# microsoft/DiskANN

Hardware: NVIDIA H100
Metric: QPS @ recall@10>=0.95, 1Mx128 f32 L2 (Vamana R=64 greedy search, batch 10K) (higher is better)
Workload: dtype f32

## Files before the change

### diskann_b200/csrc/search_common.cuh

```cuda
#pragma once

#include "distance_device.cuh"

namespace dab {

constexpr uint32_t kEmptyV2 = 0xFFFFFFFFu;
constexpr uint32_t kFlagV2 = 0x80000000u;

__device__ __forceinline__ uint32_t bucket_of(uint32_t id, uint32_t n_buckets) { return __umulhi(id * 0x9E3779B1u, n_buckets); }


__device__ __forceinline__ uint32_t first_unvisited(const uint32_t* qi, uint32_t from, uint32_t lim, int lane) {
    for (uint32_t b = from & ~31u; b < lim; b += 32) {
        const uint32_t i = b + lane;
        const bool u = i >= from && i < lim && !(qi[i] & kFlagV2);
        const unsigned m = __ballot_sync(kFull, u);
        if (m) return b + __ffs(m) - 1;
    }
    return lim;
}

template <int QT>
__device__ __forceinline__ void merge_round(float* qd, uint32_t* qi, uint32_t cap, uint32_t& size, uint32_t& cursor_lo,
                                            const uint32_t* cid, const float* cd, uint32_t c0, uint32_t m, int lane) {
    const uint32_t j = (uint32_t)lane;
    const float dj = j < m ? cd[c0 + j] : __int_as_float(0x7FC00000);
    const uint32_t idj = j < m ? cid[c0 + j] : 0;
    const float worst = size == cap ? qd[cap - 1] : __int_as_float(0x7F800000);
    const bool valid = j < m && dj == dj && !(worst < dj);
    const unsigned vm = __ballot_sync(kFull, valid);
    if (!vm) return;
    uint32_t lo = 0, hi = size;
    while (__any_sync(kFull, lo < hi)) {
        const uint32_t mid = (lo + hi) >> 1;
        if (lo < hi) {
            if (qd[mid] < dj) lo = mid + 1;
            else hi = mid;
        }
    }
    float od[QT];
    uint32_t oi[QT], sh[QT];
#pragma unroll
    for (int t = 0; t < QT; ++t) {
        const uint32_t e = (uint32_t)t * 32 + lane;
        od[t] = e < size ? qd[e] : __int_as_float(0x7F800000);
        oi[t] = e < size ? qi[e] : kEmptyV2;
        sh[t] = 0;
    }
    uint32_t rn = 0;
    unsigned it = vm;
    while (it) {
        const int i = __ffs(it) - 1;
        it &= it - 1;
        const float di = __shfl_sync(kFull, dj, i);
        rn += (di < dj || (di == dj && (uint32_t)i > j)) ? 1u : 0u;
#pragma unroll
        for (int t = 0; t < QT; ++t) sh[t] += di <= od[t] ? 1u : 0u;
    }
    const uint32_t pos = lo + rn;
    const bool keep_new = valid && pos < cap;
    __syncwarp();
#pragma unroll
    for (int t = 0; t < QT; ++t) {
        const uint32_t e = (uint32_t)t * 32 + lane;
        const uint32_t ne = e + sh[t];
        if (e < size && sh[t] != 0 && ne < cap) {
            qd[ne] = od[t];
            qi[ne] = oi[t];
        }
    }
    if (keep_new) {
        qd[pos] = dj;
        qi[pos] = idj;
    }
    size = min(cap, size + (uint32_t)__popc(vm));
    cursor_lo = min(cursor_lo, __reduce_min_sync(kFull, keep_new ? pos : 0xFFFFFFFFu));
    __syncwarp();
}

template <int QT>
__device__ __forceinline__ void merge_round_chunked(float* qd, uint32_t* qi, uint32_t cap, uint32_t& size, uint32_t& cursor_lo,
                                                    const uint32_t* cid, const float* cd, uint32_t c0, uint32_t m, int lane) {
    const uint32_t j = (uint32_t)lane;
    const float dj = j < m ? cd[c0 + j] : __int_as_float(0x7FC00000);
    const uint32_t idj = j < m ? cid[c0 + j] : 0;
    const float worst = size == cap ? qd[cap - 1] : __int_as_float(0x7F800000);
    const bool valid = j < m && dj == dj && !(worst < dj);
    const unsigned vm = __ballot_sync(kFull, valid);
    if (!vm) return;
    uint32_t lo = 0, hi = size;
    while (__any_sync(kFull, lo < hi)) {
        const uint32_t mid = (lo + hi) >> 1;
        if (lo < hi) {
            if (qd[mid] < dj) lo = mid + 1;
            else hi = mid;
        }
    }
    uint32_t rn = 0;
    for (unsigned it = vm; it;) {
        const int i = __ffs(it) - 1;
        it &= it - 1;
        const float di = __shfl_sync(kFull, dj, i);
        rn += (di < dj || (di == dj && (uint32_t)i > j)) ? 1u : 0u;
    }
    const uint32_t pos = lo + rn;
    const bool keep_new = valid && pos < cap;
    __syncwarp();
#pragma unroll 1
    for (uint32_t c = (size + QT * 32 - 1) / (QT * 32); c-- > 0;) {
        const uint32_t e0 = c * QT * 32;
        float od[QT];
        uint32_t oi[QT], sh[QT];
#pragma unroll
        for (int t = 0; t < QT; ++t) {
            const uint32_t e = e0 + (uint32_t)t * 32 + lane;
            od[t] = e < size ? qd[e] : __int_as_float(0x7F800000);
            oi[t] = e < size ? qi[e] : kEmptyV2;
            sh[t] = 0;
        }
        for (unsigned it = vm; it;) {
            const int i = __ffs(it) - 1;
            it &= it - 1;
            const float di = __shfl_sync(kFull, dj, i);
#pragma unroll
            for (int t = 0; t < QT; ++t) sh[t] += di <= od[t] ? 1u : 0u;
        }
        __syncwarp();
#pragma unroll
        for (int t = 0; t < QT; ++t) {
            const uint32_t e = e0 + (uint32_t)t * 32 + lane;
            const uint32_t ne = e + sh[t];
            if (e < size && sh[t] != 0 && ne < cap) {
                qd[ne] = od[t];
                qi[ne] = oi[t];
            }
        }
        __syncwarp();
    }
    if (keep_new) {
        qd[pos] = dj;
        qi[pos] = idj;
    }
    size = min(cap, size + (uint32_t)__popc(vm));
    cursor_lo = min(cursor_lo, __reduce_min_sync(kFull, keep_new ? pos : 0xFFFFFFFFu));
    __syncwarp();
}

template <int QT>
__device__ __forceinline__ void merge_any(float* qd, uint32_t* qi, uint32_t cap, uint32_t& size, uint32_t& cursor_lo, const uint32_t* cid,
                                          const float* cd, uint32_t c0, uint32_t m, int lane) {
    if constexpr (QT == 0) merge_round_chunked<8>(qd, qi, cap, size, cursor_lo, cid, cd, c0, m, lane);
    else if constexpr (QT == 32) merge_round_chunked<16>(qd, qi, cap, size, cursor_lo, cid, cd, c0, m, lane);
    else merge_round<QT>(qd, qi, cap, size, cursor_lo, cid, cd, c0, m, lane);
}


__device__ __forceinline__ uint64_t l2_evict_last_policy() {
    uint64_t pol;
    asm("createpolicy.fractional.L2::evict_last.b64 %0, 1.0;" : "=l"(pol));
    return pol;
}

__device__ __forceinline__ void load_bucket(const uint32_t* bp, uint32_t (&s)[8]) {
    const uint64_t pol = l2_evict_last_policy();
    asm volatile("ld.relaxed.gpu.global.L2::cache_hint.v4.b32 {%0,%1,%2,%3}, [%4], %5;"
                 : "=r"(s[0]), "=r"(s[1]), "=r"(s[2]), "=r"(s[3])
                 : "l"(bp), "l"(pol));
    asm volatile("ld.relaxed.gpu.global.L2::cache_hint.v4.b32 {%0,%1,%2,%3}, [%4], %5;"
                 : "=r"(s[4]), "=r"(s[5]), "=r"(s[6]), "=r"(s[7])
                 : "l"(bp + 4), "l"(pol));
}

__device__ __forceinline__ void store_empty_bucket(uint32_t* bp) {
    const uint64_t pol = l2_evict_last_policy();
    asm volatile("st.global.L2::cache_hint.v4.b32 [%0], {%1,%1,%1,%1}, %2;" ::"l"(bp), "r"(kEmptyV2), "l"(pol) : "memory");
    asm volatile("st.global.L2::cache_hint.v4.b32 [%0], {%1,%1,%1,%1}, %2;" ::"l"(bp + 4), "r"(kEmptyV2), "l"(pol) : "memory");
}

__device__ __forceinline__ bool bucket_insert(uint32_t* table, uint32_t n_buckets, uint32_t b, uint32_t (&s)[8], uint32_t id) {
    for (uint32_t advanced = 0;;) {
        bool found = false;
        int empty = -1;
#pragma unroll
        for (int k = 7; k >= 0; --k) {
            found |= s[k] == id;
            if (s[k] == kEmptyV2) empty = k;
        }
        if (found) return false;
        uint32_t* bp = table + (size_t)b * 8;
        if (empty >= 0) {
            const uint32_t old = atomicCAS(bp + empty, kEmptyV2, id);
            if (old == kEmptyV2) return true;
            if (old == id) return false;
        } else {
            if (++advanced > n_buckets) return false;
            b = b + 1 == n_buckets ? 0 : b + 1;
            bp = table + (size_t)b * 8;
        }
        load_bucket(bp, s);
    }
}

struct Tag16Map {
    uint32_t kmask;
    uint32_t nbk;
    uint32_t magic;
    uint32_t shift;
};

__device__ __forceinline__ void tag16_of(uint32_t id, const Tag16Map& m, uint32_t& bucket, uint32_t& tag) {
    const uint32_t h = (id * 0x9E3779B1u) & m.kmask;
    tag = (uint32_t)(((uint64_t)h * m.magic) >> m.shift);
    bucket = h - tag * m.nbk;
}


__device__ __forceinline__ int tag16_probe(uint32_t* table, uint32_t n_buckets, uint32_t b, uint32_t tag, bool allow_insert) {
    uint32_t d = 0;
    for (;;) {
        uint32_t* bp = table + (size_t)b * 8;
        const uint4 lo = reinterpret_cast<const uint4*>(bp)[0];
        const uint4 hi = reinterpret_cast<const uint4*>(bp)[1];
        const uint32_t s[8] = {lo.x, lo.y, lo.z, lo.w, hi.x, hi.y, hi.z, hi.w};
        const uint32_t want = (d << 14) | tag, want2 = want * 0x10001u;
        uint32_t hit = 0;
#pragma unroll
        for (int k = 0; k < 8; ++k) {
            const uint32_t x = s[k] ^ want2;
            hit |= (x - 0x00010001u) & ~x & 0x80008000u;
        }
        if (hit) return 0;
        int ew = -1;
        uint32_t old = 0;
#pragma unroll
        for (int k = 7; k >= 0; --k) {
            if ((s[k] >> 16) == 0xFFFFu) {
                ew = k;
                old = s[k];
            }
        }
        if (ew >= 0) {
            if (!allow_insert) return 2;
            const uint32_t neu = (old & 0xFFFFu) == 0xFFFFu ? (0xFFFF0000u | want) : ((old & 0xFFFFu) | (want << 16));
            if (atomicCAS(bp + ew, old, neu) == old) return 1;
            continue;
        }
        if (++d > 2) return 2;
        b = b + 1 == n_buckets ? 0 : b + 1;
    }
}

}
```

### diskann_b200/csrc/search_kernel_v2.cu

```cuda
#include "dab_common.cuh"
#include "distance_device.cuh"
#include "search_common.cuh"
#include "search_smem.cuh"
#include "search_v2.cuh"

#include <algorithm>
#include <cstdlib>
#include <type_traits>

namespace dab {

constexpr int kGroup = 8;
constexpr int kRowsInFlight = 4;
constexpr int kV2MinCtas = 21;
constexpr int kV2MinCtasAny = 20;
constexpr int kV2MinCtasReg = 28;

__device__ __forceinline__ void prefetch_l2(const void* p) { asm volatile("prefetch.global.L2 [%0];" ::"l"(p)); }

template <int M>
__device__ __forceinline__ void bfly8(float (&v)[kGroup], int lane, int bit) {
    const bool up = (lane & bit) != 0;
#pragma unroll
    for (int i = 0; i < M / 2; ++i) {
        const float keep = up ? v[M / 2 + i] : v[i];
        const float send = up ? v[i] : v[M / 2 + i];
        v[i] = __fadd_rn(keep, __shfl_xor_sync(kFull, send, bit));
    }
}

template <typename TD, int KIND>
__device__ __forceinline__ float group_distance(const float* __restrict__ q, const uint8_t* __restrict__ rows,
                                                uint32_t row_slot, int dim, int lane) {
    const int full8 = dim & ~7, rem = dim & 7;
    float v[kGroup];
#pragma unroll
    for (int g = 0; g < kGroup; ++g) v[g] = 0.0f;
    for (int e = lane; e < full8; e += 32) {
        const float x = q[e];
#pragma unroll
        for (int g = 0; g < kGroup; ++g) {
            const float y = to_f32(reinterpret_cast<const TD*>(rows + (size_t)g * row_slot)[e]);
            if (KIND == KIND_L2) {
                const float c = __fsub_rn(x, y);
                v[g] = __fmaf_rn(c, c, v[g]);
            } else {
                v[g] = __fmaf_rn(x, y, v[g]);
            }
        }
    }
    bfly8<8>(v, lane, 8);
    bfly8<4>(v, lane, 16);
    if (rem) {
        const int hi = (((lane >> 4) & 1) << 1) | (((lane >> 3) & 1) << 2);
        const int l = lane & 7;
#pragma unroll
        for (int i = 0; i < 2; ++i) {
            const int g = i | hi;
            const float x = l < rem ? q[full8 + l] : 0.0f;
            const float y = l < rem ? to_f32(reinterpret_cast<const TD*>(rows + (size_t)g * row_slot)[full8 + l]) : 0.0f;
            if (KIND == KIND_L2) {
                const float c = __fsub_rn(x, y);
                v[i] = __fmaf_rn(c, c, v[i]);
            } else {
                v[i] = __fmaf_rn(x, y, v[i]);
            }
        }
    }
    bfly8<2>(v, lane, 4);
    float a = v[0];
    a = __fadd_rn(a, __shfl_xor_sync(kFull, a, 2));
    a = __fadd_rn(a, __shfl_xor_sync(kFull, a, 1));
    return a;
}

template <typename T>
struct V2Int {
    static constexpr bool value = false, is_signed = false;
};
template <>
struct V2Int<int8_t> {
    static constexpr bool value = true, is_signed = true;
};
template <>
struct V2Int<uint8_t> {
    static constexpr bool value = true, is_signed = false;
};

template <bool SIGNED, int KIND>
__device__ __forceinline__ void group_distance_int(const uint8_t* __restrict__ q, const uint8_t* __restrict__ rows, uint32_t row_slot, int dim,
                                                   int lane, int qq, float (&out)[kGroup]) {
    int xy[kGroup], yy[kGroup];
#pragma unroll
    for (int g = 0; g < kGroup; ++g) xy[g] = yy[g] = 0;
    const int nwords = dim >> 2;
    for (int w = lane; w < nwords; w += 32) {
        const int x = reinterpret_cast<const int*>(q)[w];
#pragma unroll
        for (int g = 0; g < kGroup; ++g) {
            const int y = reinterpret_cast<const int*>(rows + (size_t)g * row_slot)[w];
            xy[g] = dp4<SIGNED>(x, y, xy[g]);
            if (KIND != KIND_IP) yy[g] = dp4<SIGNED>(y, y, yy[g]);
        }
    }
    const int tail = dim & 3;
    if (lane < tail) {
        const int i = (nwords << 2) + lane;
        const int x = byte_at<SIGNED>(q, i);
#pragma unroll
        for (int g = 0; g < kGroup; ++g) {
            const int y = byte_at<SIGNED>(rows + (size_t)g * row_slot, i);
            xy[g] += x * y;
            if (KIND != KIND_IP) yy[g] += y * y;
        }
    }
#pragma unroll
    for (int g = 0; g < kGroup; ++g) {
        const int sxy = __reduce_add_sync(kFull, xy[g]);
        if (KIND == KIND_IP) {
            out[g] = (float)sxy;
        } else {
            const int syy = __reduce_add_sync(kFull, yy[g]);
            if (KIND == KIND_L2) out[g] = (float)(int)((unsigned)qq + (unsigned)syy - 2u * (unsigned)sxy);
            else out[g] = cosine_finish((float)qq, (float)syy, (float)sxy);
        }
    }
}

__device__ __forceinline__ void clear_global_table(uint32_t* table, uint32_t nbk, int lane) {
#pragma unroll 1
    for (uint32_t i = lane; i < nbk; i += 32) store_empty_bucket(table + (size_t)i * 8);
    __syncwarp();
}
__device__ __forceinline__ bool global_table_insert(uint32_t* table, uint32_t nbk, uint32_t id) {
    uint32_t bs[8];
    const uint32_t b = bucket_of(id, nbk);
    load_bucket(table + (size_t)b * 8, bs);
    return bucket_insert(table, nbk, b, bs, id);
}

template <typename TD, int KIND, int POST, int QT, bool L1, bool REG>
__global__ void __launch_bounds__(kV2Warps * 32, REG ? kV2MinCtasReg : QT == 0 ? kV2MinCtasAny : kV2MinCtas) search_kernel_v2(const SearchParamsV2 p) {
    static_assert(!REG || (std::is_same<TD, float>::value && L1), "the register row path reads f32 rows, with level 1 on");
    static_assert(QT != 0 || !L1, "lists of any length run the global table alone");
    static_assert(QT == 0 || KIND != KIND_COS || V2Int<TD>::value, "float cosine reads its rows from global memory");
    extern __shared__ __align__(128) uint8_t smem[];
    const int lane = threadIdx.x & 31, wib = threadIdx.x >> 5;
    uint8_t* base = smem + (size_t)wib * p.warp_smem;
    float* qf = reinterpret_cast<float*>(base + p.off_q);
    float* qd = reinterpret_cast<float*>(base + p.off_qd);
    uint32_t* qi = reinterpret_cast<uint32_t*>(base + p.off_qi);
    uint32_t* cid = reinterpret_cast<uint32_t*>(base + p.off_cid);
    float* cd = reinterpret_cast<float*>(base + p.off_cd);
    uint32_t* beam_ids = reinterpret_cast<uint32_t*>(base + p.off_beam);
    uint32_t* adjbuf = reinterpret_cast<uint32_t*>(base + p.off_adj);
    const uint32_t adjbuf_a = smem_addr(adjbuf);

    uint32_t* t1 = reinterpret_cast<uint32_t*>(base + p.off_t1);
    const uint32_t nb1 = p.t1_buckets;
    const Tag16Map tmap{p.tag_kmask, nb1, p.tag_magic, p.tag_shift};

    const uint32_t warp_slot = blockIdx.x * kV2Warps + wib;
    const uint32_t nbk = p.n_buckets;
    uint32_t* table = p.tables + (size_t)warp_slot * nbk * 8;
    const uint32_t hlimit = nbk * 7;
    const uint64_t n_total = p.n_points + p.n_start;
    const int dim = (int)p.dim;
    uint64_t row_policy;
    asm volatile("createpolicy.fractional.L2::evict_first.b64 %0, 1.0;" : "=l"(row_policy));

    for (;;) {
        uint32_t w = 0;
        if (lane == 0) w = atomicAdd(p.counters, 1u);
        w = __shfl_sync(kFull, w, 0);
        if (w >= p.n_work) break;
        const uint32_t qidx = p.query_list ? p.query_list[w] : w;

        __syncwarp();
        {
            const TD* s = p.query_rows ? reinterpret_cast<const TD*>(p.vectors + (size_t)p.query_rows[qidx] * p.row_stride)
                                       : reinterpret_cast<const TD*>(p.queries) + (size_t)qidx * dim;
            if constexpr (V2Int<TD>::value) {
                uint8_t* qb = reinterpret_cast<uint8_t*>(qf);
                const int qbytes = (dim + 3) & ~3;
                for (int e = lane; e < qbytes; e += 32) qb[e] = e < dim ? reinterpret_cast<const uint8_t*>(s)[e] : 0;
            } else {
                for (int e = lane; e < dim; e += 32) qf[e] = to_f32(s[e]);
            }
            if constexpr (L1) {
                const uint4 e4 = make_uint4(kEmptyV2, kEmptyV2, kEmptyV2, kEmptyV2);
                for (uint32_t i = lane; i < nb1 * 2; i += 32) reinterpret_cast<uint4*>(t1)[i] = e4;
            } else {
                for (uint32_t i = lane; i < nbk; i += 32) store_empty_bucket(table + (size_t)i * 8);
            }
        }
        __syncwarp();
        int qq = 0;
        if constexpr (V2Int<TD>::value) {
            if (KIND != KIND_IP) qq = warp_int_self<V2Int<TD>::is_signed>(reinterpret_cast<const uint8_t*>(qf), dim, lane);
        }

        uint32_t size = 0, cursor_lo = 0, cmps = 0, nvisited = 0, nrec = 0;
        uint32_t n1 = 0;
        bool closed = false;
        bool l2_used = false;
        uint32_t pred = kEmptyV2;
        bool overflow = false;

        auto visit_l1 = [&](uint32_t id, bool ok) -> bool {
            bool ins = false, need = false;
            if (ok) {
                uint32_t b1, tg;
                tag16_of(id, tmap, b1, tg);
                const int r = tag16_probe(t1, nb1, b1, tg, !closed);
                ins = r == 1;
                need = r == 2;
            }
            n1 += __popc(__ballot_sync(kFull, ins));
            if (__any_sync(kFull, need)) {
                if (!l2_used) {
                    clear_global_table(table, nbk, lane);
                    l2_used = true;
                }
                bool ins2 = false;
                if (need) ins2 = global_table_insert(table, nbk, id);
                nvisited += __popc(__ballot_sync(kFull, ins2));
                ins |= ins2;
            }
            return ins;
        };


        auto stage = [&](uint32_t c0, uint32_t n) {
            uint8_t* rows = base + p.off_rows;
            const uint32_t rows_a = smem_addr(rows);
            const uint32_t sub = (uint32_t)lane >> 3, nsub = 4, off0 = ((uint32_t)lane & 7u) * 16u, offs = 128;
            auto copy16 = [&](uint32_t dst, const uint8_t* src) {
                asm volatile("cp.async.cg.shared.global.L2::cache_hint [%0], [%1], 16, %2;" ::"r"(dst), "l"(src), "l"(row_policy) : "memory");
            };
            auto issue = [&](uint32_t lo, uint32_t hi) {
                if (p.row_bytes == 4 * offs) {
                    for (uint32_t j = lo + sub; j < hi; j += nsub) {
                        const uint8_t* src = p.vectors + (size_t)cid[c0 + j] * p.row_stride + off0;
                        const uint32_t dst = rows_a + j * p.row_slot + off0;
#pragma unroll
                        for (uint32_t k = 0; k < 4; ++k) copy16(dst + k * offs, src + k * offs);
                    }
                } else {
                    for (uint32_t j = lo + sub; j < hi; j += nsub) {
                        const uint8_t* src = p.vectors + (size_t)cid[c0 + j] * p.row_stride;
                        const uint32_t dst = rows_a + j * p.row_slot;
                        for (uint32_t off = off0; off < p.row_bytes; off += offs) copy16(dst + off, src + off);
                    }
                }
                asm volatile("cp.async.commit_group;" ::: "memory");
            };
            auto compute = [&](uint32_t g0) {
                if constexpr (V2Int<TD>::value) {
                    float vals[kGroup];
                    group_distance_int<V2Int<TD>::is_signed, KIND>(reinterpret_cast<const uint8_t*>(qf), rows + (size_t)g0 * p.row_slot,
                                                                  p.row_slot, dim, lane, qq, vals);
#pragma unroll
                    for (int u = 0; u < kGroup; ++u)
                        if (lane == u && g0 + u < n) cd[c0 + g0 + u] = post_op<POST>(vals[u]);
                } else {
                    const float r = group_distance<TD, KIND>(qf, rows + (size_t)g0 * p.row_slot, p.row_slot, dim, lane);
                    const uint32_t u = (((lane >> 3) & 1) << 2) | (((lane >> 4) & 1) << 1) | ((lane >> 2) & 1);
                    if ((lane & 3) == 0 && g0 + u < n) cd[c0 + g0 + u] = post_op<POST>(r);
                }
            };
            issue(0, n);
            asm volatile("cp.async.wait_group 0;" ::: "memory");
            __syncwarp();
            for (uint32_t g0 = 0; g0 < n; g0 += kGroup) compute(g0);
            __syncwarp();
        };

        auto distances = [&](uint32_t n) {
            if constexpr (REG) {
                const int nm = dim >> 5;
                uint64_t q2[8] = {0ull, 0ull, 0ull, 0ull, 0ull, 0ull, 0ull, 0ull};
#pragma unroll
                for (int m = 0; m < 4; ++m) {
                    if (m < nm) {
                        const float4 x = *reinterpret_cast<const float4*>(qf + 32 * m + 4 * (lane & 7));
                        q2[2 * m] = pack2(x.x, x.y);
                        q2[2 * m + 1] = pack2(x.z, x.w);
                    }
                }
                wide_distances_f32_fast<KIND, POST>(q2, nm, p.vectors, p.row_stride, cid, n, cd, lane);
                __syncwarp();
            } else if constexpr (QT == 0) {
                constexpr bool INT = V2Int<TD>::value;
                constexpr int S = KIND == KIND_COS && !INT ? 16 : 32, TEAMS = 32 / S, U = kRowsInFlight;
                using Row = typename std::conditional<INT, uint8_t, TD>::type;
                const int team = lane / S, slot = lane % S;
                for (uint32_t c0 = 0; c0 < n; c0 += TEAMS * U) {
                    float r[U];
                    uint32_t cc[U];
                    const Row* rows[U];
#pragma unroll
                    for (int u = 0; u < U; ++u) {
                        cc[u] = c0 + u * TEAMS + team;
                        rows[u] = reinterpret_cast<const Row*>(p.vectors + (size_t)cid[min(cc[u], n - 1)] * p.row_stride);
                    }
                    if constexpr (INT) warp_int_multi<V2Int<TD>::is_signed, KIND, U>(reinterpret_cast<const uint8_t*>(qf), rows, dim, lane, qq, r);
                    else team_float_multi<S / 8, KIND, U>(qf, rows, dim, slot, r);
#pragma unroll
                    for (int u = 0; u < U; ++u)
                        if (slot == 0 && cc[u] < n) cd[cc[u]] = post_op<POST>(r[u]);
                }
                __syncwarp();
            } else {
                for (uint32_t c0 = 0; c0 < n; c0 += p.stage_rows) stage(c0, min(p.stage_rows, n - c0));
            }
        };

        for (uint32_t s0 = 0; s0 < p.n_start; s0 += 32) {
            const uint32_t n = min(32u, p.n_start - s0);
            if constexpr (L1) {
                const uint32_t id = (uint32_t)p.n_points + s0 + lane;
                if ((uint32_t)lane < n) cid[lane] = id;
                visit_l1(id, (uint32_t)lane < n);
            } else if ((uint32_t)lane < n) {
                const uint32_t id = (uint32_t)p.n_points + s0 + lane;
                cid[lane] = id;
                uint32_t bs[8];
                const uint32_t b = bucket_of(id, nbk);
                load_bucket(table + (size_t)b * 8, bs);
                bucket_insert(table, nbk, b, bs, id);
            }
            __syncwarp();
            distances(n);
            merge_any<QT>(qd, qi, p.cap, size, cursor_lo, cid, cd, 0, n, lane);
            if constexpr (!L1) nvisited += n;
            cmps += n;
        }

        for (;;) {
            const uint32_t lim = min(p.cap, size);
            uint32_t nb = 0;
            while (nb < p.beam) {
                const uint32_t idx = first_unvisited(qi, cursor_lo, lim, lane);
                if (idx >= lim) break;
                const uint32_t id = qi[idx];
                __syncwarp();
                if (lane == 0) {
                    qi[idx] = id | kFlagV2;
                    beam_ids[nb] = id;
                    if (p.rec_ids && nrec < p.rec_cap) {
                        p.rec_ids[(size_t)qidx * p.rec_cap + nrec] = id;
                        p.rec_dists[(size_t)qidx * p.rec_cap + nrec] = qd[idx];
                    }
                }
                cursor_lo = idx + 1;
                ++nrec;
                ++nb;
                __syncwarp();
            }
            if (nb == 0) break;

            uint32_t ncand = 0;
            for (uint32_t b = 0; b < nb; ++b) {
                const uint32_t node = beam_ids[b];
                const uint32_t* row = p.adj + (size_t)node * p.adj_stride;
                uint32_t wd[3];
                if (b == 0 && p.adj_words) {
                    asm volatile("cp.async.wait_group 0;" ::: "memory");
                    __syncwarp();
                }
                if (b == 0 && node == pred) {
                    wd[0] = adjbuf[lane];
                    wd[1] = 32 + lane < p.adj_words ? adjbuf[32 + lane] : kEmptyV2;
                    wd[2] = 64 + lane < p.adj_words ? adjbuf[64 + lane] : kEmptyV2;
                    __syncwarp();
                } else {
                    wd[0] = __ldg(row + lane);
                    wd[1] = 32 + lane < p.adj_stride ? __ldg(row + 32 + lane) : kEmptyV2;
                    wd[2] = 64 + lane < p.adj_stride ? __ldg(row + 64 + lane) : kEmptyV2;
                }
                if (b == 0) {
                    const uint32_t nxt = first_unvisited(qi, cursor_lo, lim, lane);
                    pred = kEmptyV2;
                    if (nxt < lim) {
                        const uint32_t nid = qi[nxt] & ~kFlagV2;
                        const uint32_t* nrow = p.adj + (size_t)nid * p.adj_stride;
                        if (p.adj_words) {
                            pred = nid;
                            if ((uint32_t)lane * 4 < p.adj_words)
                                asm volatile("cp.async.cg.shared.global [%0], [%1], 16;" ::"r"(adjbuf_a + lane * 16), "l"(nrow + lane * 4)
                                             : "memory");
                            asm volatile("cp.async.commit_group;" ::: "memory");
                        } else if (lane < 3) {
                            prefetch_l2(nrow + lane * 32);
                        }
                    }
                }
                const uint32_t deg = min(__shfl_sync(kFull, wd[0], 0), p.max_degree);
                if constexpr (L1) {
#pragma unroll 1
                    for (uint32_t c0 = 0; c0 <= deg; c0 += 32) {
                        const uint32_t j = c0 + lane;
                        uint32_t word = c0 == 0 ? wd[0] : (c0 == 32 ? wd[1] : wd[2]);
                        if (c0 >= 96) word = j < p.adj_stride ? __ldg(row + j) : kEmptyV2;
                        const bool ins = visit_l1(word, j >= 1 && j <= deg);
                        const bool isnew = ins && word < n_total;
                        const unsigned mn = __ballot_sync(kFull, isnew);
                        if (isnew) cid[ncand + __popc(mn & ((1u << lane) - 1u))] = word;
                        ncand += __popc(mn);
                    }
                    if (!closed && n1 + p.max_degree > p.t1_limit) closed = true;
                } else {
                    bool valid[3];
                    uint32_t bk[3];
                    uint32_t bs[3][8];
#pragma unroll
                    for (int c = 0; c < 3; ++c) {
                        const uint32_t j = c * 32 + lane;
                        valid[c] = j >= 1 && j <= deg;
                        bk[c] = bucket_of(wd[c], nbk);
                        if (valid[c]) load_bucket(table + (size_t)bk[c] * 8, bs[c]);
                    }
#pragma unroll
                    for (int c = 0; c < 3; ++c) {
                        bool inserted = false;
                        if (valid[c]) inserted = bucket_insert(table, nbk, bk[c], bs[c], wd[c]);
                        const bool isnew = inserted && wd[c] < n_total;
                        const unsigned mi = __ballot_sync(kFull, inserted);
                        const unsigned mn = __ballot_sync(kFull, isnew);
                        if (isnew) cid[ncand + __popc(mn & ((1u << lane) - 1u))] = wd[c];
                        ncand += __popc(mn);
                        nvisited += __popc(mi);
                    }
                    for (uint32_t c0 = 96; c0 < deg + 1; c0 += 32) {
                        const uint32_t j = c0 + lane;
                        const uint32_t word = j < p.adj_stride ? __ldg(row + j) : kEmptyV2;
                        bool inserted = false;
                        if (j <= deg) {
                            const uint32_t b2 = bucket_of(word, nbk);
                            uint32_t bs2[8];
                            load_bucket(table + (size_t)b2 * 8, bs2);
                            inserted = bucket_insert(table, nbk, b2, bs2, word);
                        }
                        const bool isnew = inserted && word < n_total;
                        const unsigned mi = __ballot_sync(kFull, inserted);
                        const unsigned mn = __ballot_sync(kFull, isnew);
                        if (isnew) cid[ncand + __popc(mn & ((1u << lane) - 1u))] = word;
                        ncand += __popc(mn);
                        nvisited += __popc(mi);
                    }
                }
                if (nvisited + p.max_degree > hlimit) {
                    overflow = true;
                    break;
                }
            }
            if (overflow) break;
            __syncwarp();

            distances(ncand);

            for (uint32_t c0 = 0; c0 < ncand; c0 += 32)
                merge_any<QT>(qd, qi, p.cap, size, cursor_lo, cid, cd, c0, min(32u, ncand - c0), lane);
            cmps += ncand;
        }

        if (overflow) {
            if (lane == 0) {
                uint32_t o = atomicAdd(p.counters + 1, 1u);
                p.overflow_list[o] = qidx;
            }
            continue;
        }

        {
            const uint32_t n = min(p.cap, size);
            uint32_t count = 0;
            for (uint32_t b = 0; b < n && count < p.k; b += 32) {
                const uint32_t i = b + lane;
                const uint32_t id = i < n ? (qi[i] & ~kFlagV2) : kEmptyV2;
                const bool keep = i < n && id < p.n_points;
                const unsigned m = __ballot_sync(kFull, keep);
                const uint32_t pos = count + __popc(m & ((1u << lane) - 1u));
                if (keep && pos < p.k) {
                    p.out_ids[(size_t)qidx * p.k + pos] = id;
                    p.out_dists[(size_t)qidx * p.k + pos] = qd[i];
                }
                count += __popc(m);
            }
            count = min(count, p.k);
            for (uint32_t i = count + lane; i < p.k; i += 32) {
                p.out_ids[(size_t)qidx * p.k + i] = kEmptyV2;
                p.out_dists[(size_t)qidx * p.k + i] = __int_as_float(0x7F800000);
            }
            if (lane == 0) {
                atomicMax(p.counters + 2, n1 + nvisited);
                if (p.out_counts) p.out_counts[qidx] = count;
                if (p.out_cmps) p.out_cmps[qidx] = cmps;
                if (p.out_hops) p.out_hops[qidx] = nrec;
                if (p.rec_counts) {
                    p.rec_counts[qidx] = min(nrec, p.rec_cap);
                    if (nrec > p.rec_cap) atomicAdd(p.counters + 3, 1u);
                }
            }
        }
    }
    if constexpr (REG) asm volatile("cp.async.wait_group 0;" ::: "memory");
}

template <typename TD, int K, int P, int Q>
static void (*pick_v2(bool l1, bool reg))(const SearchParamsV2) {
    if constexpr (std::is_same<TD, float>::value) {
        if (reg) return search_kernel_v2<TD, K, P, Q, true, true>;
    }
    return l1 ? search_kernel_v2<TD, K, P, Q, true, false> : search_kernel_v2<TD, K, P, Q, false, false>;
}

template <typename S>
static int v2_prepare_schema(const dab_index* idx, uint32_t l_search, uint32_t beam, bool level1, SearchParamsV2& p, V2Launch& out) {
    const uint32_t cap = l_search + idx->n_start;
    const uint32_t row_bytes = (uint32_t)round_up((size_t)idx->dim * elem_size(idx->dtype), 16);
    auto too_big = [&] {
        return fail(DAB_ERR_INVALID_ARGUMENT, "search: L=%u, beam=%u, dim=%u need %zu B shared memory per CTA (> 200 KB)", l_search,
                    beam, idx->dim, out.smem_block);
    };
    size_t off = 0;
    p.off_q = (uint32_t)off;
    off += S::IS_INT ? round_up(round_up((size_t)idx->dim, 4), 16) : round_up((size_t)idx->dim * 4, 16);
    const size_t ncand_max = (size_t)beam * idx->max_degree;
    p.off_cid = (uint32_t)off;
    off += round_up(std::max<size_t>(ncand_max, idx->n_start) * 4, 16);
    p.off_cd = (uint32_t)off;
    off += round_up(std::max<size_t>(ncand_max, idx->n_start) * 4, 16);
    p.off_beam = (uint32_t)off;
    off += round_up((size_t)beam * 4, 16);
    p.adj_words = idx->adj_stride % 4 == 0 ? (uint32_t)std::min<size_t>(idx->adj_stride, 96) : 0;
    p.off_adj = (uint32_t)off;
    off += (size_t)p.adj_words * 4;
    const size_t cap_pad = round_up(cap, 4);
    p.off_qd = (uint32_t)off;
    off += cap_pad * 4;
    p.off_qi = (uint32_t)off;
    off += cap_pad * 4;
    p.row_bytes = row_bytes;
    const size_t stage_bytes = 6144;
    const uint32_t stage = std::min<uint32_t>(32, (uint32_t)std::max<size_t>(kGroup, (stage_bytes / row_bytes) / kGroup * kGroup));
    const bool any_len = cap > 256 || S::NA == 2 || round_up(off, 128) + (size_t)stage * row_bytes > 200 * 1024;
    size_t t1_bytes = idx->tune.test_visited_log2 ? 512 : 4096;
    p.t1_buckets = 0;
    uint32_t K = 8;
    while (((uint64_t)1 << K) < idx->n_total()) ++K;
    const uint64_t nb1 = t1_bytes / 32;
    uint32_t sbits = 0;
    while (((uint64_t)1 << sbits) < nb1) ++sbits;
    if ((((uint64_t)1 << K) + 16383) >> 14 <= nb1 && K + sbits <= 32) {
        p.t1_buckets = (uint32_t)nb1;
        p.t1_limit = (uint32_t)(nb1 * 14);
        p.tag_kmask = (uint32_t)(((uint64_t)1 << K) - 1);
        p.tag_shift = K + sbits;
        p.tag_magic = (uint32_t)((((uint64_t)1 << (K + sbits)) + nb1 - 1) / nb1);
    }
    if (!level1 || any_len) p.t1_buckets = 0;
    auto resident_warps = [&](size_t t1_at) {
        return (227 * 1024) / (round_up(round_up(t1_at, 32) + t1_bytes, 128) * kV2Warps + 1024) * kV2Warps;
    };
    const bool reg = idx->dtype == DAB_F32 && idx->dim % 32 == 0 && idx->dim <= 128 && p.t1_buckets && resident_warps(off) >= 16;
    if (!reg && !any_len) {
        off = round_up(off, 128);
        p.off_rows = (uint32_t)off;
        p.stage_rows = stage;
        p.row_slot = row_bytes;
        off += (size_t)stage * row_bytes;
    }
    p.off_t1 = (uint32_t)round_up(off, 32);
    if (p.t1_buckets && resident_warps(off) < 16) p.t1_buckets = 0;
    if (!p.t1_buckets) t1_bytes = 0;
    p.warp_smem = (uint32_t)round_up((size_t)p.off_t1 + t1_bytes, 128);
    out.smem_block = (size_t)p.warp_smem * kV2Warps;
    if (out.smem_block > 200 * 1024) return too_big();

    using TD = typename S::TD;
    const bool l1 = p.t1_buckets != 0;
    if (any_len) out.kern = search_kernel_v2<TD, S::KIND, S::POST, 0, false, false>;
    else if constexpr (S::NA == 4)
        out.kern = cap <= 128 ? pick_v2<TD, S::KIND, S::POST, 4>(l1, reg) : pick_v2<TD, S::KIND, S::POST, 8>(l1, reg);
    int per_sm = 0;
    if (cudaFuncSetAttribute(out.kern, cudaFuncAttributeMaxDynamicSharedMemorySize, (int)out.smem_block) != cudaSuccess ||
        cudaOccupancyMaxActiveBlocksPerMultiprocessor(&per_sm, out.kern, kV2Warps * 32, out.smem_block) != cudaSuccess || per_sm < 1) {
        cudaGetLastError();
        return too_big();
    }
    out.grid = per_sm * idx->sm_count;
    return 0;
}

int v2_prepare(const dab_index* idx, uint32_t l_search, uint32_t beam, bool level1, SearchParamsV2& p, V2Launch& out) {
    return visit_schema<OPS_QUERY>(idx->dtype, idx->metric, [&](auto s) {
        return v2_prepare_schema<decltype(s)>(idx, l_search, beam, level1, p, out);
    });
}

}
```

### diskann_b200/csrc/search_smem.cuh

```cuda
#pragma once

#include "distance_device.cuh"
#include "search_common.cuh"

namespace dab {
namespace {

__device__ __forceinline__ uint32_t smem_addr(const void* p) { return (uint32_t)__cvta_generic_to_shared(p); }

__device__ __forceinline__ void load_bucket_smem(const uint32_t* bp, uint32_t (&s)[8]) {
    const uint4 lo = reinterpret_cast<const uint4*>(bp)[0];
    const uint4 hi = reinterpret_cast<const uint4*>(bp)[1];
    s[0] = lo.x, s[1] = lo.y, s[2] = lo.z, s[3] = lo.w, s[4] = hi.x, s[5] = hi.y, s[6] = hi.z, s[7] = hi.w;
}

__device__ __forceinline__ bool smem16_insert(uint32_t* table, uint32_t n_buckets, uint32_t b, uint32_t tag, bool& ovf) {
    uint32_t d = 0;
    for (;;) {
        uint32_t* bp = table + (size_t)b * 8;
        uint32_t s[8];
        load_bucket_smem(bp, s);
        const uint32_t want = (d << 14) | tag, want2 = want * 0x10001u;
        uint32_t hit = 0;
#pragma unroll
        for (int k = 0; k < 8; ++k) {
            const uint32_t x = s[k] ^ want2;
            hit |= (x - 0x00010001u) & ~x & 0x80008000u;
        }
        if (hit) return false;
        int ew = -1;
        uint32_t old = 0;
#pragma unroll
        for (int k = 7; k >= 0; --k) {
            if ((s[k] >> 16) == 0xFFFFu) {
                ew = k;
                old = s[k];
            }
        }
        if (ew >= 0) {
            const uint32_t neu = (old & 0xFFFFu) == 0xFFFFu ? (0xFFFF0000u | want) : ((old & 0xFFFFu) | (want << 16));
            if (atomicCAS(bp + ew, old, neu) == old) return true;
            continue;
        }
        if (++d > 2) {
            ovf = true;
            return false;
        }
        b = b + 1 == n_buckets ? 0 : b + 1;
    }
}

__device__ __forceinline__ uint64_t pack2(float lo, float hi) {
    uint64_t r;
    asm("mov.b64 %0, {%1, %2};" : "=l"(r) : "f"(lo), "f"(hi));
    return r;
}
__device__ __forceinline__ void unpack2(uint64_t v, float& lo, float& hi) { asm("mov.b64 {%0, %1}, %2;" : "=f"(lo), "=f"(hi) : "l"(v)); }
template <int KIND>
__device__ __forceinline__ uint64_t step2(uint64_t acc, uint64_t x2, uint64_t y2) {
    float a0, a1, x0, x1, y0, y1;
    unpack2(acc, a0, a1);
    unpack2(x2, x0, x1);
    unpack2(y2, y0, y1);
    if (KIND == KIND_L2) {
        const float c0 = __fsub_rn(x0, y0), c1 = __fsub_rn(x1, y1);
        a0 = __fmaf_rn(c0, c0, a0);
        a1 = __fmaf_rn(c1, c1, a1);
    } else {
        a0 = __fmaf_rn(x0, y0, a0);
        a1 = __fmaf_rn(x1, y1, a1);
    }
    return pack2(a0, a1);
}

__device__ __forceinline__ uint4 ldg16(const uint8_t* p) { return __ldg(reinterpret_cast<const uint4*>(p)); }

__device__ __forceinline__ void prefetch_rows(const uint8_t* __restrict__ vectors, size_t row_stride, const uint32_t* __restrict__ cid,
                                              uint32_t n, uint32_t row_bytes16, int lane) {
    for (uint32_t j = lane; j < n; j += 32) {
        const uint8_t* src = vectors + (size_t)cid[j] * row_stride;
        asm volatile("cp.async.bulk.prefetch.L2.global [%0], %1;" ::"l"(src), "r"(row_bytes16) : "memory");
    }
}

template <int KIND, int POST>
__device__ __forceinline__ void wide_distances_f32_fast(const uint64_t (&q2)[8], int nm, const uint8_t* __restrict__ vectors,
                                                        size_t row_stride, const uint32_t* __restrict__ cid, uint32_t n,
                                                        float* __restrict__ cd, int lane) {
    const int team = lane >> 3, tl = lane & 7;
    if (n > 4) prefetch_rows(vectors, row_stride, cid, n, (uint32_t)nm * 128u, lane);
    for (uint32_t j0 = 0; j0 < n; j0 += 4) {
        const uint8_t* row0 = vectors + (size_t)cid[min(j0 + team, n - 1)] * row_stride + 16 * tl;
        uint4 v0[4];
#pragma unroll
        for (int m = 0; m < 4; ++m)
            if (m < nm) v0[m] = ldg16(row0 + m * 128);
        uint64_t a0[2] = {0ull, 0ull};
#pragma unroll
        for (int m = 0; m < 4; ++m) {
            if (m < nm) {
                a0[0] = step2<KIND>(a0[0], q2[2 * m], pack2(__uint_as_float(v0[m].x), __uint_as_float(v0[m].y)));
                a0[1] = step2<KIND>(a0[1], q2[2 * m + 1], pack2(__uint_as_float(v0[m].z), __uint_as_float(v0[m].w)));
            }
        }
        float acc[4];
        unpack2(a0[0], acc[0], acc[1]);
        unpack2(a0[1], acc[2], acc[3]);
#pragma unroll
        for (int i = 0; i < 4; ++i) {
            acc[i] = __fadd_rn(acc[i], __shfl_xor_sync(kFull, acc[i], 2));
            acc[i] = __fadd_rn(acc[i], __shfl_xor_sync(kFull, acc[i], 4));
        }
        float ts[4];
#pragma unroll
        for (int i = 0; i < 4; ++i) ts[i] = __fadd_rn(acc[i], __shfl_xor_sync(kFull, acc[i], 1));
        const float r = __fadd_rn(__fadd_rn(ts[0], ts[2]), __fadd_rn(ts[1], ts[3]));
        if (tl == 0 && j0 + team < n) cd[j0 + team] = post_op<POST>(r);
    }
}


template <typename TD, int KIND, int POST, int P, int U>
__device__ __forceinline__ void wide_distances(const float* __restrict__ q, const uint8_t* __restrict__ vectors, size_t row_stride,
                                               const uint32_t* __restrict__ cid, uint32_t n, float* __restrict__ cd, int dim, int lane) {
    constexpr int EPL = 16 / (int)sizeof(TD), LPR = 32 / EPL, ROWS = EPL, HALVES = 8 / EPL;
    const int team = lane / LPR, tl = lane % LPR;
    const int a = tl / HALVES, h = tl % HALVES;
    const int nb8 = dim >> 3, full8 = dim & ~7, rem = dim & 7;
    const int nm = (nb8 + 3) >> 2;
    if (n > P * ROWS) prefetch_rows(vectors, row_stride, cid, n, (uint32_t)((dim * (int)sizeof(TD) + 15) & ~15), lane);
    for (uint32_t j0 = 0; j0 < n; j0 += P * ROWS) {
        const uint8_t* row[P];
        bool act[P];
#pragma unroll
        for (int pp = 0; pp < P; ++pp) {
            act[pp] = j0 + pp * ROWS < n;
            const uint32_t jj = min(j0 + pp * ROWS + team, n - 1);
            row[pp] = vectors + (size_t)cid[jj] * row_stride + 16 * tl;
        }
        uint64_t acc2[P][EPL / 2];
#pragma unroll
        for (int pp = 0; pp < P; ++pp)
#pragma unroll
            for (int i = 0; i < EPL / 2; ++i) acc2[pp][i] = 0ull;
        for (int m0 = 0; m0 < nm; m0 += U) {
            uint4 v[P][U];
#pragma unroll
            for (int pp = 0; pp < P; ++pp) {
                if (act[pp]) {
#pragma unroll
                    for (int u = 0; u < U; ++u)
                        if (a + 4 * (m0 + u) < nb8) v[pp][u] = ldg16(row[pp] + (size_t)(m0 + u) * (LPR * 16));
                }
            }
#pragma unroll
            for (int u = 0; u < U; ++u) {
                if (a + 4 * (m0 + u) < nb8) {
                    const float* qx = q + ((m0 + u) * (LPR * 16) + 16 * tl) / (int)sizeof(TD);
                    float4 x[EPL / 4];
#pragma unroll
                    for (int i = 0; i < EPL / 4; ++i) x[i] = reinterpret_cast<const float4*>(qx)[i];
#pragma unroll
                    for (int pp = 0; pp < P; ++pp) {
                        if (act[pp]) {
                            if constexpr (sizeof(TD) == 2) {
                                const __half2* hp = reinterpret_cast<const __half2*>(&v[pp][u]);
                                const float2 f0 = __half22float2(hp[0]), f1 = __half22float2(hp[1]);
                                const float2 f2 = __half22float2(hp[2]), f3 = __half22float2(hp[3]);
                                acc2[pp][0] = step2<KIND>(acc2[pp][0], pack2(x[0].x, x[0].y), pack2(f0.x, f0.y));
                                acc2[pp][1] = step2<KIND>(acc2[pp][1], pack2(x[0].z, x[0].w), pack2(f1.x, f1.y));
                                acc2[pp][2] = step2<KIND>(acc2[pp][2], pack2(x[1].x, x[1].y), pack2(f2.x, f2.y));
                                acc2[pp][3] = step2<KIND>(acc2[pp][3], pack2(x[1].z, x[1].w), pack2(f3.x, f3.y));
                            } else {
                                const uint4 w = v[pp][u];
                                acc2[pp][0] = step2<KIND>(acc2[pp][0], pack2(x[0].x, x[0].y),
                                                          pack2(__uint_as_float(w.x), __uint_as_float(w.y)));
                                acc2[pp][1] = step2<KIND>(acc2[pp][1], pack2(x[0].z, x[0].w),
                                                          pack2(__uint_as_float(w.z), __uint_as_float(w.w)));
                            }
                        }
                    }
                }
            }
        }
#pragma unroll
        for (int pp = 0; pp < P; ++pp) {
            if (!act[pp]) continue;
            float acc[EPL];
#pragma unroll
            for (int i = 0; i < EPL / 2; ++i) unpack2(acc2[pp][i], acc[2 * i], acc[2 * i + 1]);
#pragma unroll
            for (int i = 0; i < EPL; ++i) {
                acc[i] = __fadd_rn(acc[i], __shfl_xor_sync(kFull, acc[i], HALVES));
                acc[i] = __fadd_rn(acc[i], __shfl_xor_sync(kFull, acc[i], 2 * HALVES));
            }
            if (rem) {
                const TD* tail = reinterpret_cast<const TD*>(row[pp] - 16 * tl) + full8;
#pragma unroll
                for (int i = 0; i < EPL; ++i) {
                    const int l = EPL * h + i;
                    const float x = l < rem ? q[full8 + l] : 0.0f;
                    const float yv = l < rem ? ldg_elem(tail + l) : 0.0f;
                    if (KIND == KIND_L2) {
                        const float dd = __fsub_rn(x, yv);
                        acc[i] = __fmaf_rn(dd, dd, acc[i]);
                    } else {
                        acc[i] = __fmaf_rn(x, yv, acc[i]);
                    }
                }
            }
            float r;
            if constexpr (HALVES == 1) {
                r = __fadd_rn(__fadd_rn(__fadd_rn(acc[0], acc[4]), __fadd_rn(acc[2], acc[6])),
                              __fadd_rn(__fadd_rn(acc[1], acc[5]), __fadd_rn(acc[3], acc[7])));
            } else {
                float ts[4];
#pragma unroll
                for (int i = 0; i < 4; ++i) ts[i] = __fadd_rn(acc[i], __shfl_xor_sync(kFull, acc[i], 1));
                r = __fadd_rn(__fadd_rn(ts[0], ts[2]), __fadd_rn(ts[1], ts[3]));
            }
            const uint32_t jj = j0 + pp * ROWS + team;
            if (tl == 0 && jj < n) cd[jj] = post_op<POST>(r);
        }
    }
}

template <bool SIGNED, int KIND, int POST, int P>
__device__ __forceinline__ void wide_distances_int(const uint8_t* __restrict__ q, int qq, const uint8_t* __restrict__ vectors,
                                                   size_t row_stride, const uint32_t* __restrict__ cid, uint32_t n,
                                                   float* __restrict__ cd, int dim, int lane) {
    constexpr int ROWS = 4;
    const int team = lane >> 3, tl = lane & 7;
    const int nfull = dim >> 4, tail = dim & 15;
    const int nm = (nfull + 7) >> 3;
    if (n > P * ROWS) prefetch_rows(vectors, row_stride, cid, n, (uint32_t)((dim + 15) & ~15), lane);
    for (uint32_t j0 = 0; j0 < n; j0 += P * ROWS) {
        const uint8_t* row[P];
        bool act[P];
        int xy[P], yy[P];
#pragma unroll
        for (int pp = 0; pp < P; ++pp) {
            act[pp] = j0 + pp * ROWS < n;
            const uint32_t jj = min(j0 + pp * ROWS + team, n - 1);
            row[pp] = vectors + (size_t)cid[jj] * row_stride;
            xy[pp] = yy[pp] = 0;
        }
        for (int m = 0; m < nm; ++m) {
            const int c = m * 8 + tl;
            if (c < nfull) {
                uint4 v[P];
#pragma unroll
                for (int pp = 0; pp < P; ++pp)
                    if (act[pp]) v[pp] = ldg16(row[pp] + (size_t)c * 16);
                const uint4 x = reinterpret_cast<const uint4*>(q)[c];
#pragma unroll
                for (int pp = 0; pp < P; ++pp) {
                    if (act[pp]) {
                        xy[pp] = dp4<SIGNED>((int)x.x, (int)v[pp].x, xy[pp]);
                        xy[pp] = dp4<SIGNED>((int)x.y, (int)v[pp].y, xy[pp]);
                        xy[pp] = dp4<SIGNED>((int)x.z, (int)v[pp].z, xy[pp]);
                        xy[pp] = dp4<SIGNED>((int)x.w, (int)v[pp].w, xy[pp]);
                        if (KIND != KIND_IP) {
                            yy[pp] = dp4<SIGNED>((int)v[pp].x, (int)v[pp].x, yy[pp]);
                            yy[pp] = dp4<SIGNED>((int)v[pp].y, (int)v[pp].y, yy[pp]);
                            yy[pp] = dp4<SIGNED>((int)v[pp].z, (int)v[pp].z, yy[pp]);
                            yy[pp] = dp4<SIGNED>((int)v[pp].w, (int)v[pp].w, yy[pp]);
                        }
                    }
                }
            }
        }
        if (tail) {
#pragma unroll
            for (int t = 0; t < 2; ++t) {
                const int i = (nfull << 4) + tl * 2 + t;
                if (tl * 2 + t < tail) {
                    const int x = byte_at<SIGNED>(q, i);
#pragma unroll
                    for (int pp = 0; pp < P; ++pp) {
                        if (act[pp]) {
                            const int y = SIGNED ? (int)(int8_t)__ldg(row[pp] + i) : (int)__ldg(row[pp] + i);
                            xy[pp] += x * y;
                            if (KIND != KIND_IP) yy[pp] += y * y;
                        }
                    }
                }
            }
        }
#pragma unroll
        for (int pp = 0; pp < P; ++pp) {
            if (!act[pp]) continue;
            int sxy = xy[pp], syy = yy[pp];
#pragma unroll
            for (int o = 4; o >= 1; o >>= 1) {
                sxy += __shfl_xor_sync(kFull, sxy, o);
                if (KIND != KIND_IP) syy += __shfl_xor_sync(kFull, syy, o);
            }
            float r;
            if (KIND == KIND_IP) r = (float)sxy;
            else if (KIND == KIND_L2) r = (float)(int)((unsigned)qq + (unsigned)syy - 2u * (unsigned)sxy);
            else r = cosine_finish((float)qq, (float)syy, (float)sxy);
            const uint32_t jj = j0 + pp * ROWS + team;
            if (tl == 0 && jj < n) cd[jj] = post_op<POST>(r);
        }
    }
}

}
}
```

### diskann_b200/csrc/search_v2.cuh

```cuda
#pragma once

#include "dab_common.cuh"

namespace dab {

constexpr int kV2Warps = 1;

struct SearchParamsV2 {
    const uint8_t* vectors;
    size_t row_stride;
    const uint32_t* adj;
    uint32_t adj_stride;
    uint64_t n_points;
    uint32_t n_start;
    uint32_t dim;
    uint32_t max_degree;
    const void* queries;
    const uint32_t* query_rows;
    const uint32_t* query_list;
    uint32_t n_work;
    uint32_t k, cap, beam;
    uint32_t* out_ids;
    float* out_dists;
    uint32_t* out_counts;
    uint32_t* out_cmps;
    uint32_t* out_hops;
    uint32_t* tables;
    uint32_t n_buckets;
    uint32_t t1_buckets;
    uint32_t t1_limit;
    uint32_t tag_kmask, tag_magic, tag_shift, off_t1;
    uint32_t* counters;
    uint32_t* overflow_list;
    uint32_t* rec_ids;
    float* rec_dists;
    uint32_t* rec_counts;
    uint32_t rec_cap;
    uint32_t warp_smem, off_q, off_qd, off_qi, off_cid, off_cd, off_beam, off_rows, off_adj;
    uint32_t adj_words;
    uint32_t row_bytes;
    uint32_t row_slot;
    uint32_t stage_rows;
};

struct V2Launch {
    void (*kern)(const SearchParamsV2);
    size_t smem_block;
    int grid;
};

int v2_prepare(const dab_index* idx, uint32_t l_search, uint32_t beam, bool level1, SearchParamsV2& p, V2Launch& out);

}
```

Before: 4.662 million.

## Streamline search inner loop: fused rank, two-unvisited scan, pow2 tags, line prefetch

Four separate micro-changes to the greedy search loop. The merge round now derives each candidate's insertion position from the existing compare loop with a warp reduce instead of a separate binary search, and one scan now finds both the next and the following unvisited entry. The level-1 tag hash uses shift/mask for power-of-two bucket counts instead of a magic multiply, so that table is now disabled when the bucket count is not a power of two. Row prefetch issues per-128B-line L2 prefetches spread across lanes instead of one bulk prefetch per row.

Result: no change. 4.648 million (median of 6 runs) (-0.3%).

```diff
diff --git a/diskann_b200/csrc/search_common.cuh b/diskann_b200/csrc/search_common.cuh
--- a/diskann_b200/csrc/search_common.cuh
+++ b/diskann_b200/csrc/search_common.cuh
@@ -18,6 +18,25 @@
         if (m) return b + __ffs(m) - 1;
     }
     return lim;
+}
+
+__device__ __forceinline__ uint32_t first_two_unvisited(const uint32_t* qi, uint32_t from, uint32_t lim, int lane, uint32_t& second) {
+    uint32_t first = lim;
+    for (uint32_t b = from & ~31u; b < lim; b += 32) {
+        const uint32_t i = b + lane;
+        const bool u = i >= from && i < lim && !(qi[i] & kFlagV2);
+        unsigned m = __ballot_sync(kFull, u);
+        if (first == lim && m) {
+            first = b + __ffs(m) - 1;
+            m &= m - 1;
+        }
+        if (m) {
+            second = b + __ffs(m) - 1;
+            return first;
+        }
+    }
+    second = lim;
+    return first;
 }
 
 template <int QT>
@@ -30,14 +49,6 @@
     const bool valid = j < m && dj == dj && !(worst < dj);
     const unsigned vm = __ballot_sync(kFull, valid);
     if (!vm) return;
-    uint32_t lo = 0, hi = size;
-    while (__any_sync(kFull, lo < hi)) {
-        const uint32_t mid = (lo + hi) >> 1;
-        if (lo < hi) {
-            if (qd[mid] < dj) lo = mid + 1;
-            else hi = mid;
-        }
-    }
     float od[QT];
     uint32_t oi[QT], sh[QT];
 #pragma unroll
@@ -47,15 +58,22 @@
         oi[t] = e < size ? qi[e] : kEmptyV2;
         sh[t] = 0;
     }
-    uint32_t rn = 0;
+    uint32_t rn = 0, lo = 0;
     unsigned it = vm;
     while (it) {
         const int i = __ffs(it) - 1;
         it &= it - 1;
         const float di = __shfl_sync(kFull, dj, i);
         rn += (di < dj || (di == dj && (uint32_t)i > j)) ? 1u : 0u;
-#pragma unroll
-        for (int t = 0; t < QT; ++t) sh[t] += di <= od[t] ? 1u : 0u;
+        uint32_t ge = 0;
+#pragma unroll
+        for (int t = 0; t < QT; ++t) {
+            const uint32_t le = di <= od[t] ? 1u : 0u;
+            sh[t] += le;
+            ge += le;
+        }
+        const uint32_t below = QT * 32 - __reduce_add_sync(kFull, ge);
+        if ((uint32_t)i == j) lo = below;
     }
     const uint32_t pos = lo + rn;
     const bool keep_new = valid && pos < cap;
@@ -214,6 +232,12 @@
     bucket = h - tag * m.nbk;
 }
 
+__device__ __forceinline__ void tag16_of_pow2(uint32_t id, uint32_t kmask, uint32_t log2_nbk, uint32_t& bucket, uint32_t& tag) {
+    const uint32_t h = (id * 0x9E3779B1u) & kmask;
+    tag = h >> log2_nbk;
+    bucket = h & ((1u << log2_nbk) - 1u);
+}
+
 
 __device__ __forceinline__ int tag16_probe(uint32_t* table, uint32_t n_buckets, uint32_t b, uint32_t tag, bool allow_insert) {
     uint32_t d = 0;
diff --git a/diskann_b200/csrc/search_kernel_v2.cu b/diskann_b200/csrc/search_kernel_v2.cu
--- a/diskann_b200/csrc/search_kernel_v2.cu
+++ b/diskann_b200/csrc/search_kernel_v2.cu
@@ -158,7 +158,6 @@
 
     uint32_t* t1 = reinterpret_cast<uint32_t*>(base + p.off_t1);
     const uint32_t nb1 = p.t1_buckets;
-    const Tag16Map tmap{p.tag_kmask, nb1, p.tag_magic, p.tag_shift};
 
     const uint32_t warp_slot = blockIdx.x * kV2Warps + wib;
     const uint32_t nbk = p.n_buckets;
@@ -211,7 +210,7 @@
             bool ins = false, need = false;
             if (ok) {
                 uint32_t b1, tg;
-                tag16_of(id, tmap, b1, tg);
+                tag16_of_pow2(id, p.tag_kmask, p.t1_log2, b1, tg);
                 const int r = tag16_probe(t1, nb1, b1, tg, !closed);
                 ins = r == 1;
                 need = r == 2;
@@ -340,8 +339,9 @@
         for (;;) {
             const uint32_t lim = min(p.cap, size);
             uint32_t nb = 0;
+            uint32_t nxt = lim;
             while (nb < p.beam) {
-                const uint32_t idx = first_unvisited(qi, cursor_lo, lim, lane);
+                const uint32_t idx = first_two_unvisited(qi, cursor_lo, lim, lane, nxt);
                 if (idx >= lim) break;
                 const uint32_t id = qi[idx];
                 __syncwarp();
@@ -380,7 +380,6 @@
                     wd[2] = 64 + lane < p.adj_stride ? __ldg(row + 64 + lane) : kEmptyV2;
                 }
                 if (b == 0) {
-                    const uint32_t nxt = first_unvisited(qi, cursor_lo, lim, lane);
                     pred = kEmptyV2;
                     if (nxt < lim) {
                         const uint32_t nid = qi[nxt] & ~kFlagV2;
@@ -553,12 +552,11 @@
     const uint64_t nb1 = t1_bytes / 32;
     uint32_t sbits = 0;
     while (((uint64_t)1 << sbits) < nb1) ++sbits;
-    if ((((uint64_t)1 << K) + 16383) >> 14 <= nb1 && K + sbits <= 32) {
+    if ((((uint64_t)1 << K) + 16383) >> 14 <= nb1 && K + sbits <= 32 && nb1 == ((uint64_t)1 << sbits)) {
         p.t1_buckets = (uint32_t)nb1;
         p.t1_limit = (uint32_t)(nb1 * 14);
         p.tag_kmask = (uint32_t)(((uint64_t)1 << K) - 1);
-        p.tag_shift = K + sbits;
-        p.tag_magic = (uint32_t)((((uint64_t)1 << (K + sbits)) + nb1 - 1) / nb1);
+        p.t1_log2 = sbits;
     }
     if (!level1 || any_len) p.t1_buckets = 0;
     auto resident_warps = [&](size_t t1_at) {
diff --git a/diskann_b200/csrc/search_smem.cuh b/diskann_b200/csrc/search_smem.cuh
--- a/diskann_b200/csrc/search_smem.cuh
+++ b/diskann_b200/csrc/search_smem.cuh
@@ -76,10 +76,13 @@
 __device__ __forceinline__ uint4 ldg16(const uint8_t* p) { return __ldg(reinterpret_cast<const uint4*>(p)); }
 
 __device__ __forceinline__ void prefetch_rows(const uint8_t* __restrict__ vectors, size_t row_stride, const uint32_t* __restrict__ cid,
-                                              uint32_t n, uint32_t row_bytes16, int lane) {
-    for (uint32_t j = lane; j < n; j += 32) {
+                                              uint32_t n, uint32_t row_bytes, int lane) {
+    const uint32_t lines = (row_bytes + 127) >> 7;
+    const uint32_t lg = lines >= 32 ? 5u : 32u - (uint32_t)__clz(lines - 1);
+    const uint32_t per = 1u << lg, l0 = (uint32_t)lane & (per - 1);
+    for (uint32_t j = (uint32_t)lane >> lg; j < n; j += 32u >> lg) {
         const uint8_t* src = vectors + (size_t)cid[j] * row_stride;
-        asm volatile("cp.async.bulk.prefetch.L2.global [%0], %1;" ::"l"(src), "r"(row_bytes16) : "memory");
+        for (uint32_t l = l0; l < lines; l += per) asm volatile("prefetch.global.L2 [%0];" ::"l"(src + 128 * l));
     }
 }
 
diff --git a/diskann_b200/csrc/search_v2.cuh b/diskann_b200/csrc/search_v2.cuh
--- a/diskann_b200/csrc/search_v2.cuh
+++ b/diskann_b200/csrc/search_v2.cuh
@@ -29,7 +29,7 @@
     uint32_t n_buckets;
     uint32_t t1_buckets;
     uint32_t t1_limit;
-    uint32_t tag_kmask, tag_magic, tag_shift, off_t1;
+    uint32_t tag_kmask, t1_log2, off_t1;
     uint32_t* counters;
     uint32_t* overflow_list;
     uint32_t* rec_ids;
```
